# OpenRobotLab/EmbodiedScan

Hardware: NVIDIA H100
Metric: training scans/sec mv-3ddet 20-view (ResNet-50/16 + MinkResNet34, 480x640, 100k pts) (higher is better)
Workload: dtype bf16

## Files before the change

### embodiedscan_b200/csrc/common.cuh

```cuda
#pragma once
#include <cuda_runtime.h>
#include <cuda_bf16.h>
#include <stdint.h>
#include <stdio.h>
#include <stdarg.h>
#include "../../include/esb200.h"

void esb_set_error(const char* fmt, ...);

#define ESB_CHECK_ARG(cond, ...)                      \
  do {                                                \
    if (!(cond)) {                                    \
      esb_set_error(__VA_ARGS__);                     \
      return ESB_EINVAL;                              \
    }                                                 \
  } while (0)

#define ESB_CUDA_LAUNCH_CHECK(name)                                        \
  do {                                                                     \
    cudaError_t _e = cudaPeekAtLastError();                                \
    if (_e != cudaSuccess) {                                               \
      esb_set_error("%s: CUDA error %s", name, cudaGetErrorString(_e));    \
      return ESB_ECUDA;                                                    \
    }                                                                      \
  } while (0)

#define ESB_CUDA_CALL(expr)                                                \
  do {                                                                     \
    cudaError_t _e = (expr);                                               \
    if (_e != cudaSuccess) {                                               \
      esb_set_error("%s: CUDA error %s", #expr, cudaGetErrorString(_e));   \
      return ESB_ECUDA;                                                    \
    }                                                                      \
  } while (0)

static inline int esb_div_up(long long a, long long b) { return (int)((a + b - 1) / b); }
static inline size_t esb_align(size_t x, size_t a = 256) { return (x + a - 1) / a * a; }
cudaError_t esb_scratch_alloc(void** p, size_t bytes, cudaStream_t s);
cudaError_t esb_scratch_free(void* p, cudaStream_t s);
int esb_sum_partial_rows(const float* part, int n_parts, long long width, float* out, int accumulate, cudaStream_t s);

int esb_sm_count();

template <int MODE>
__device__ __forceinline__ float esb_cd_crit(float x) {
  if constexpr (MODE == ESB_CD_L1) {
    return fabsf(x);
  } else if constexpr (MODE == ESB_CD_L2) {
    return __fmul_rn(x, x);
  } else {
    const float a = fabsf(x);
    return a < 1.f ? __fmul_rn(0.5f * a, a) : a - 0.5f;
  }
}
template <int MODE>
__device__ __forceinline__ float esb_cd_dcrit(float x) {
  if constexpr (MODE == ESB_CD_L1) {
    return x > 0.f ? 1.f : (x < 0.f ? -1.f : 0.f);
  } else if constexpr (MODE == ESB_CD_L2) {
    return 2.f * x;
  } else {
    return fminf(fmaxf(x, -1.f), 1.f);
  }
}


#define ESB_EMPTY_KEY 0xFFFFFFFFFFFFFFFFull
#define ESB_COORD_BIAS 32768

__host__ __device__ __forceinline__ uint64_t esb_pack_key(int b, int x, int y, int z) {
  return ((uint64_t)(uint16_t)b << 48) | ((uint64_t)(uint16_t)(x + ESB_COORD_BIAS) << 32) |
         ((uint64_t)(uint16_t)(y + ESB_COORD_BIAS) << 16) | (uint64_t)(uint16_t)(z + ESB_COORD_BIAS);
}
__host__ __device__ __forceinline__ bool esb_coord_in_range(int b, int x, int y, int z) {
  return b >= 0 && b < 65535 && x >= -ESB_COORD_BIAS && x < ESB_COORD_BIAS && y >= -ESB_COORD_BIAS &&
         y < ESB_COORD_BIAS && z >= -ESB_COORD_BIAS && z < ESB_COORD_BIAS;
}
__host__ __device__ __forceinline__ uint32_t esb_hash64(uint64_t k) {
  k ^= k >> 33;
  k *= 0xff51afd7ed558ccdull;
  k ^= k >> 33;
  k *= 0xc4ceb9fe1a85ec53ull;
  k ^= k >> 33;
  return (uint32_t)k;
}

#ifdef __CUDACC__
__device__ __forceinline__ int esb_floor_div(int a, int d) {
  int q = a / d;
  return (a % d != 0 && a < 0) ? q - 1 : q;
}

__device__ __forceinline__ int esb_hash_find(const unsigned long long* __restrict__ keys,
                                             const int* __restrict__ vals, uint32_t mask, uint64_t key) {
  uint32_t slot = esb_hash64(key) & mask;
  for (uint32_t probe = 0; probe <= mask; ++probe) {
    unsigned long long k = keys[slot];
    if (k == key) return vals[slot];
    if (k == ESB_EMPTY_KEY) return -1;
    slot = (slot + 1) & mask;
  }
  return -1;
}

template <typename T>
__device__ __forceinline__ float esb_to_float(T v);
template <>
__device__ __forceinline__ float esb_to_float<float>(float v) { return v; }
template <>
__device__ __forceinline__ float esb_to_float<__nv_bfloat16>(__nv_bfloat16 v) { return __bfloat162float(v); }

template <typename T>
__device__ __forceinline__ T esb_from_float(float v);
template <>
__device__ __forceinline__ float esb_from_float<float>(float v) { return v; }
template <>
__device__ __forceinline__ __nv_bfloat16 esb_from_float<__nv_bfloat16>(float v) { return __float2bfloat16_rn(v); }

__device__ __forceinline__ float esb_warp_sum(float v) {
#pragma unroll
  for (int o = 16; o > 0; o >>= 1) v += __shfl_xor_sync(0xffffffffu, v, o);
  return v;
}
__device__ __forceinline__ float esb_warp_max(float v) {
#pragma unroll
  for (int o = 16; o > 0; o >>= 1) v = fmaxf(v, __shfl_xor_sync(0xffffffffu, v, o));
  return v;
}
#endif
```

### embodiedscan_b200/csrc/scratch.cu

```cuda
#include <mutex>

#include "common.cuh"

namespace {

__global__ void sum_partial_rows_kernel(const float* __restrict__ part, int n_parts, long long width, float* __restrict__ out,
                                        int accumulate) {
  const long long j = blockIdx.x * (long long)blockDim.x + threadIdx.x;
  if (j >= width) return;
  float s = accumulate ? out[j] : 0.f;
  for (int p = 0; p < n_parts; ++p) s += part[(long long)p * width + j];
  out[j] = s;
}

}

int esb_sm_count() {
  static int sms[64] = {};
  int dev = 0;
  cudaGetDevice(&dev);
  if (dev >= 64) return 132;
  if (sms[dev] == 0) {
    int n = 132;
    cudaDeviceGetAttribute(&n, cudaDevAttrMultiProcessorCount, dev);
    sms[dev] = n;
  }
  return sms[dev];
}

namespace {
constexpr unsigned long long kScratchKeepBytes = 512ull << 20;
std::mutex g_pool_mutex;
cudaMemPool_t g_pool[64] = {};

cudaMemPool_t scratch_pool(int dev, cudaStream_t s) {
  if (dev < 0 || dev >= 64) return nullptr;
  std::lock_guard<std::mutex> lock(g_pool_mutex);
  if (g_pool[dev] == nullptr) {
    cudaStreamCaptureStatus st = cudaStreamCaptureStatusNone;
    cudaStreamIsCapturing(s, &st);
    if (st != cudaStreamCaptureStatusNone) return nullptr;
    cudaMemPoolProps props = {};
    props.allocType = cudaMemAllocationTypePinned;
    props.location.type = cudaMemLocationTypeDevice;
    props.location.id = dev;
    cudaMemPool_t pool = nullptr;
    if (cudaMemPoolCreate(&pool, &props) != cudaSuccess) return nullptr;
    unsigned long long keep = kScratchKeepBytes;
    cudaMemPoolSetAttribute(pool, cudaMemPoolAttrReleaseThreshold, &keep);
    g_pool[dev] = pool;
  }
  return g_pool[dev];
}
}

cudaError_t esb_scratch_alloc(void** p, size_t bytes, cudaStream_t s) {
  int dev = 0;
  cudaGetDevice(&dev);
  const size_t n = bytes > 0 ? bytes : 16;
  cudaMemPool_t pool = scratch_pool(dev, s);
  return pool != nullptr ? cudaMallocFromPoolAsync(p, n, pool, s) : cudaMallocAsync(p, n, s);
}

cudaError_t esb_scratch_free(void* p, cudaStream_t s) { return cudaFreeAsync(p, s); }

int esb_sum_partial_rows(const float* part, int n_parts, long long width, float* out, int accumulate, cudaStream_t s) {
  if (width == 0) return ESB_OK;
  sum_partial_rows_kernel<<<esb_div_up(width, 256), 256, 0, s>>>(part, n_parts, width, out, accumulate);
  ESB_CUDA_LAUNCH_CHECK("sum_partial_rows_kernel");
  return ESB_OK;
}
```

### embodiedscan_b200/csrc/spops.cu

```cuda
#include "common.cuh"

namespace {

template <typename T>
__global__ void maxpool_fwd_kernel(const T* __restrict__ x, const int* __restrict__ nbr, T* __restrict__ y,
                                   int* __restrict__ arg, long long n_out, int C, int K) {
  long long t = blockIdx.x * (long long)blockDim.x + threadIdx.x;
  if (t >= n_out * C) return;
  long long o = t / C;
  int c = (int)(t - o * C);
  float best = -INFINITY;
  int best_i = -1;
  for (int k = 0; k < K; ++k) {
    int i = nbr[(long long)k * n_out + o];
    if (i < 0) continue;
    float v = esb_to_float<T>(x[(long long)i * C + c]);
    if (best_i < 0 || v > best) {
      best = v;
      best_i = i;
    }
  }
  y[t] = esb_from_float<T>(best_i >= 0 ? best : 0.f);
  arg[t] = best_i;
}

template <typename T>
__global__ void maxpool_bwd_kernel(const T* __restrict__ dy, const int* __restrict__ arg, T* __restrict__ dx,
                                   long long n_out, int C) {
  long long t = blockIdx.x * (long long)blockDim.x + threadIdx.x;
  if (t >= n_out * C) return;
  int c = (int)(t % C);
  int i = arg[t];
  if (i >= 0) dx[(long long)i * C + c] = dy[t];
}

__device__ __forceinline__ int seg_begin(const int* __restrict__ seg_off, int s) { return seg_off ? seg_off[s] : 0; }
__device__ __forceinline__ int seg_end(const int* __restrict__ seg_off, int s, int n_total) {
  return seg_off ? seg_off[s + 1] : n_total;
}

template <typename T, int MODE>
__global__ void seg_colstat_kernel(const T* __restrict__ x, const int* __restrict__ seg_off, const float* __restrict__ mean,
                                   float* __restrict__ out, int C, int rows_per_block, int n_total) {
  __shared__ float red[8][33];
  const int s = blockIdx.y;
  const int c = blockIdx.z * 32 + threadIdx.x;
  const int r_beg = seg_begin(seg_off, s) + blockIdx.x * rows_per_block;
  const int r_end = min(seg_end(seg_off, s, n_total), r_beg + rows_per_block);
  float acc = 0.f;
  if (c < C) {
    float mu = MODE == 1 ? mean[s * C + c] : 0.f;
    for (int r = r_beg + threadIdx.y; r < r_end; r += 8) {
      float v = esb_to_float<T>(x[(long long)r * C + c]);
      if (MODE == 1) {
        v -= mu;
        acc = fmaf(v, v, acc);
      } else {
        acc += v;
      }
    }
  }
  red[threadIdx.y][threadIdx.x] = acc;
  __syncthreads();
  if (threadIdx.y == 0 && c < C) {
    float t = 0.f;
#pragma unroll
    for (int j = 0; j < 8; ++j) t += red[j][threadIdx.x];
    out[((long long)blockIdx.x * gridDim.y + s) * C + c] = t;
  }
}

__global__ void seg_finalize_mean_kernel(float* __restrict__ sum, const int* __restrict__ seg_off, int S, int C,
                                         int n_total) {
  int t = blockIdx.x * blockDim.x + threadIdx.x;
  if (t >= S * C) return;
  int s = t / C;
  int n = seg_end(seg_off, s, n_total) - seg_begin(seg_off, s);
  sum[t] = n > 0 ? sum[t] / (float)n : 0.f;
}
__global__ void seg_finalize_rstd_kernel(const float* __restrict__ mean, float* __restrict__ var_to_rstd,
                                         const int* __restrict__ seg_off, int S, int C, float eps,
                                         float* __restrict__ running_mean, float* __restrict__ running_var,
                                         float momentum, int n_total) {
  int t = blockIdx.x * blockDim.x + threadIdx.x;
  if (t >= S * C) return;
  int s = t / C;
  int n = seg_end(seg_off, s, n_total) - seg_begin(seg_off, s);
  float var = n > 0 ? var_to_rstd[t] / (float)n : 0.f;
  if (running_mean != nullptr && S == 1) {
    float unbiased = n > 1 ? var * (float)n / (float)(n - 1) : var;
    running_mean[t] = (1.f - momentum) * running_mean[t] + momentum * mean[t];
    running_var[t] = (1.f - momentum) * running_var[t] + momentum * unbiased;
  }
  var_to_rstd[t] = rsqrtf(var + eps);
}

__device__ __forceinline__ float act_fwd(float z, int act) {
  if (act == 1) return fmaxf(z, 0.f);
  if (act == 2) return z > 0.f ? z : expm1f(z);
  return z;
}
__device__ __forceinline__ float act_bwd_from_out(float y, int act) {
  if (act == 1) return y > 0.f ? 1.f : 0.f;
  if (act == 2) return y > 0.f ? 1.f : y + 1.f;
  return 1.f;
}

template <typename T>
__global__ void norm_apply_kernel(const T* __restrict__ x, const T* __restrict__ res, const int* __restrict__ row_seg,
                                  const float* __restrict__ mean, const float* __restrict__ rstd,
                                  const float* __restrict__ gamma, const float* __restrict__ beta, T* __restrict__ y,
                                  long long N, int C, int act) {
  long long t = blockIdx.x * (long long)blockDim.x + threadIdx.x;
  if (t >= N * C) return;
  long long r = t / C;
  int c = (int)(t - r * C);
  int s = row_seg ? row_seg[r] : 0;
  float g = gamma ? gamma[c] : 1.f, b = beta ? beta[c] : 0.f;
  float z = (esb_to_float<T>(x[t]) - mean[s * C + c]) * rstd[s * C + c] * g + b;
  if (res) z += esb_to_float<T>(res[t]);
  y[t] = esb_from_float<T>(act_fwd(z, act));
}

template <typename T>
__device__ __forceinline__ void load8(const T* p, float v[8]);
template <>
__device__ __forceinline__ void load8<float>(const float* p, float v[8]) {
  float4 a = reinterpret_cast<const float4*>(p)[0], b = reinterpret_cast<const float4*>(p)[1];
  v[0] = a.x; v[1] = a.y; v[2] = a.z; v[3] = a.w; v[4] = b.x; v[5] = b.y; v[6] = b.z; v[7] = b.w;
}
template <>
__device__ __forceinline__ void load8<__nv_bfloat16>(const __nv_bfloat16* p, float v[8]) {
  uint4 raw = *reinterpret_cast<const uint4*>(p);
  const __nv_bfloat162* h = reinterpret_cast<const __nv_bfloat162*>(&raw);
#pragma unroll
  for (int i = 0; i < 4; ++i) { v[2 * i] = __low2float(h[i]); v[2 * i + 1] = __high2float(h[i]); }
}
template <typename T>
__device__ __forceinline__ void store8(T* p, const float v[8]);
template <>
__device__ __forceinline__ void store8<float>(float* p, const float v[8]) {
  reinterpret_cast<float4*>(p)[0] = make_float4(v[0], v[1], v[2], v[3]);
  reinterpret_cast<float4*>(p)[1] = make_float4(v[4], v[5], v[6], v[7]);
}
template <>
__device__ __forceinline__ void store8<__nv_bfloat16>(__nv_bfloat16* p, const float v[8]) {
  uint4 o;
  __nv_bfloat162* h = reinterpret_cast<__nv_bfloat162*>(&o);
#pragma unroll
  for (int i = 0; i < 4; ++i) h[i] = __floats2bfloat162_rn(v[2 * i], v[2 * i + 1]);
  *reinterpret_cast<uint4*>(p) = o;
}

template <typename T>
__global__ void norm_apply_vec8_kernel(const T* __restrict__ x, const T* __restrict__ res, const int* __restrict__ row_seg,
                                       const float* __restrict__ mean, const float* __restrict__ rstd,
                                       const float* __restrict__ gamma, const float* __restrict__ beta, T* __restrict__ y,
                                       long long n_vec, int C, int act) {
  long long t = blockIdx.x * (long long)blockDim.x + threadIdx.x;
  if (t >= n_vec) return;
  const int cv = C >> 3;
  const long long r = t / cv;
  const int c0 = (int)(t - r * cv) << 3;
  const int s = row_seg ? row_seg[r] : 0;
  float v[8], rr[8];
  load8<T>(x + t * 8, v);
  if (res) load8<T>(res + t * 8, rr);
#pragma unroll
  for (int i = 0; i < 8; ++i) {
    const int c = c0 + i;
    float z = (v[i] - mean[s * C + c]) * rstd[s * C + c] * (gamma ? gamma[c] : 1.f) + (beta ? beta[c] : 0.f);
    if (res) z += rr[i];
    v[i] = act_fwd(z, act);
  }
  store8<T>(y + t * 8, v);
}

template <typename T>
__global__ void norm_bwd_apply_vec8_kernel(const T* __restrict__ x, const T* __restrict__ y, const T* __restrict__ dy,
                                           const int* __restrict__ row_seg, const int* __restrict__ seg_off,
                                           const float* __restrict__ mean, const float* __restrict__ rstd,
                                           const float* __restrict__ gamma, const float* __restrict__ sg,
                                           const float* __restrict__ sgx, T* __restrict__ dx, T* __restrict__ dres,
                                           long long N, long long n_vec, int C, int act) {
  long long t = blockIdx.x * (long long)blockDim.x + threadIdx.x;
  if (t >= n_vec) return;
  const int cv = C >> 3;
  const long long r = t / cv;
  const int c0 = (int)(t - r * cv) << 3;
  const int s = row_seg ? row_seg[r] : 0;
  const float inv_n = 1.f / (float)max(seg_end(seg_off, s, (int)N) - seg_begin(seg_off, s), 1);
  float xv[8], yv[8], gv[8], ov[8];
  load8<T>(x + t * 8, xv);
  load8<T>(y + t * 8, yv);
  load8<T>(dy + t * 8, gv);
#pragma unroll
  for (int i = 0; i < 8; ++i) {
    const int c = c0 + i;
    float g = gv[i] * act_bwd_from_out(yv[i], act);
    float rs = rstd[s * C + c];
    float xh = (xv[i] - mean[s * C + c]) * rs;
    ov[i] = (gamma ? gamma[c] : 1.f) * rs * (g - sg[s * C + c] * inv_n - xh * sgx[s * C + c] * inv_n);
    gv[i] = g;
  }
  store8<T>(dx + t * 8, ov);
  if (dres) store8<T>(dres + t * 8, gv);
}

template <typename T>
__global__ void norm_bwd_reduce_kernel(const T* __restrict__ x, const T* __restrict__ y, const T* __restrict__ dy,
                                       const int* __restrict__ seg_off, const float* __restrict__ mean,
                                       const float* __restrict__ rstd, float* __restrict__ sg, float* __restrict__ sgx,
                                       int C, int rows_per_block, int act, int n_total) {
  __shared__ float red0[8][33];
  __shared__ float red1[8][33];
  const int s = blockIdx.y;
  const int c = blockIdx.z * 32 + threadIdx.x;
  const int r_beg = seg_begin(seg_off, s) + blockIdx.x * rows_per_block;
  const int r_end = min(seg_end(seg_off, s, n_total), r_beg + rows_per_block);
  float a0 = 0.f, a1 = 0.f;
  if (c < C) {
    float mu = mean[s * C + c], rs = rstd[s * C + c];
    for (int r = r_beg + threadIdx.y; r < r_end; r += 8) {
      long long idx = (long long)r * C + c;
      float g = esb_to_float<T>(dy[idx]) * act_bwd_from_out(esb_to_float<T>(y[idx]), act);
      float xh = (esb_to_float<T>(x[idx]) - mu) * rs;
      a0 += g;
      a1 = fmaf(g, xh, a1);
    }
  }
  red0[threadIdx.y][threadIdx.x] = a0;
  red1[threadIdx.y][threadIdx.x] = a1;
  __syncthreads();
  if (threadIdx.y == 0 && c < C) {
    float t0 = 0.f, t1 = 0.f;
#pragma unroll
    for (int j = 0; j < 8; ++j) {
      t0 += red0[j][threadIdx.x];
      t1 += red1[j][threadIdx.x];
    }
    sg[((long long)blockIdx.x * gridDim.y + s) * C + c] = t0;
    sgx[((long long)blockIdx.x * gridDim.y + s) * C + c] = t1;
  }
}

template <typename T>
__global__ void norm_bwd_apply_kernel(const T* __restrict__ x, const T* __restrict__ y, const T* __restrict__ dy,
                                      const int* __restrict__ row_seg, const int* __restrict__ seg_off,
                                      const float* __restrict__ mean, const float* __restrict__ rstd,
                                      const float* __restrict__ gamma, const float* __restrict__ sg,
                                      const float* __restrict__ sgx, T* __restrict__ dx, T* __restrict__ dres,
                                      long long N, int C, int act) {
  long long t = blockIdx.x * (long long)blockDim.x + threadIdx.x;
  if (t >= N * C) return;
  long long r = t / C;
  int c = (int)(t - r * C);
  int s = row_seg ? row_seg[r] : 0;
  float inv_n = 1.f / (float)max(seg_end(seg_off, s, (int)N) - seg_begin(seg_off, s), 1);
  float g = esb_to_float<T>(dy[t]) * act_bwd_from_out(esb_to_float<T>(y[t]), act);
  float rs = rstd[s * C + c];
  float xh = (esb_to_float<T>(x[t]) - mean[s * C + c]) * rs;
  float gm = gamma ? gamma[c] : 1.f;
  float v = gm * rs * (g - sg[s * C + c] * inv_n - xh * sgx[s * C + c] * inv_n);
  dx[t] = esb_from_float<T>(v);
  if (dres) dres[t] = esb_from_float<T>(g);
}

template <typename T>
__global__ void bias_act_kernel(const T* __restrict__ x, const float* __restrict__ bias, const T* __restrict__ res,
                                T* __restrict__ y, long long n_vec, int C, int act) {
  long long t = blockIdx.x * (long long)blockDim.x + threadIdx.x;
  if (t >= n_vec) return;
  const int cv = C / 8;
  const int c0 = (int)(t % cv) * 8;
  float v[8], r[8];
  if (sizeof(T) == 2) {
    uint4 raw = reinterpret_cast<const uint4*>(x)[t];
    const __nv_bfloat162* h = reinterpret_cast<const __nv_bfloat162*>(&raw);
#pragma unroll
    for (int i = 0; i < 4; ++i) { v[2 * i] = __low2float(h[i]); v[2 * i + 1] = __high2float(h[i]); }
    if (res) {
      uint4 rr = reinterpret_cast<const uint4*>(res)[t];
      const __nv_bfloat162* g = reinterpret_cast<const __nv_bfloat162*>(&rr);
#pragma unroll
      for (int i = 0; i < 4; ++i) { r[2 * i] = __low2float(g[i]); r[2 * i + 1] = __high2float(g[i]); }
    }
  } else {
#pragma unroll
    for (int i = 0; i < 8; ++i) { v[i] = esb_to_float<T>(x[t * 8 + i]); r[i] = res ? esb_to_float<T>(res[t * 8 + i]) : 0.f; }
  }
#pragma unroll
  for (int i = 0; i < 8; ++i) v[i] = act_fwd(v[i] + (bias ? bias[c0 + i] : 0.f) + (res ? r[i] : 0.f), act);
  if (sizeof(T) == 2) {
    uint4 o;
    __nv_bfloat162* h = reinterpret_cast<__nv_bfloat162*>(&o);
#pragma unroll
    for (int i = 0; i < 4; ++i) h[i] = __floats2bfloat162_rn(v[2 * i], v[2 * i + 1]);
    reinterpret_cast<uint4*>(y)[t] = o;
  } else {
#pragma unroll
    for (int i = 0; i < 8; ++i) y[t * 8 + i] = esb_from_float<T>(v[i]);
  }
}

template <typename T>
__global__ void act_bwd_kernel(const T* __restrict__ dy, const T* __restrict__ y, T* __restrict__ dx, long long n,
                               int act) {
  long long t = (blockIdx.x * (long long)blockDim.x + threadIdx.x) * 8;
  if (t + 8 <= n) {
    float g[8], o[8];
    load8<T>(dy + t, g);
    load8<T>(y + t, o);
#pragma unroll
    for (int i = 0; i < 8; ++i) g[i] *= act_bwd_from_out(o[i], act);
    store8<T>(dx + t, g);
  } else {
    for (int i = 0; i < 8; ++i)
      if (t + i < n)
        dx[t + i] = esb_from_float<T>(esb_to_float<T>(dy[t + i]) * act_bwd_from_out(esb_to_float<T>(y[t + i]), act));
  }
}

template <typename T>
__global__ void bn_stats_kernel(const T* __restrict__ x, long long N, int C, int rows_per_block, float* __restrict__ part) {
  extern __shared__ float sh[];
  const int tpr = C / 8;
  const int c = (threadIdx.x % tpr) * 8;
  const int rsub = threadIdx.x / tpr, rstep = blockDim.x / tpr;
  const long long r_beg = (long long)blockIdx.x * rows_per_block;
  const long long r_end = r_beg + rows_per_block < N ? r_beg + rows_per_block : N;
  float piv[8], sum[8], sq[8];
  load8<T>(x + c, piv);
#pragma unroll
  for (int e = 0; e < 8; ++e) sum[e] = sq[e] = 0.f;
  if (rsub < rstep) {
    for (long long r = r_beg + rsub; r < r_end; r += rstep) {
      float v[8];
      load8<T>(x + r * C + c, v);
#pragma unroll
      for (int e = 0; e < 8; ++e) {
        const float d = v[e] - piv[e];
        sum[e] += d;
        sq[e] = fmaf(d, d, sq[e]);
      }
    }
#pragma unroll
    for (int e = 0; e < 8; ++e) {
      sh[(2 * rsub) * C + c + e] = sum[e];
      sh[(2 * rsub + 1) * C + c + e] = sq[e];
    }
  }
  __syncthreads();
  for (int i = threadIdx.x; i < 2 * C; i += blockDim.x) {
    const int k = i < C ? 0 : 1, ci = i < C ? i : i - C;
    float t = 0.f;
    for (int r = 0; r < rstep; ++r) t += sh[(2 * r + k) * C + ci];
    part[(long long)blockIdx.x * 2 * C + i] = t;
  }
}

template <typename T>
__global__ void bn_apply_fused_kernel(const T* __restrict__ x, const T* __restrict__ res, long long N, int C,
                                      const float* __restrict__ gamma, const float* __restrict__ beta, float eps,
                                      float* __restrict__ running_mean, float* __restrict__ running_var, float momentum, int act,
                                      float* __restrict__ stats, T* __restrict__ y) {
  const float inv_n = 1.f / (float)N;
  if (blockIdx.x == 0) {
    for (int i = threadIdx.x; i < C; i += blockDim.x) {
      const float m = stats[i] * inv_n;
      const float var = fmaxf(stats[C + i] * inv_n - m * m, 0.f);
      const float mean = esb_to_float<T>(x[i]) + m;
      stats[2 * C + i] = mean;
      stats[3 * C + i] = rsqrtf(var + eps);
      if (running_mean != nullptr) {
        const float unbiased = N > 1 ? var * (float)N / (float)(N - 1) : var;
        running_mean[i] = (1.f - momentum) * running_mean[i] + momentum * mean;
        running_var[i] = (1.f - momentum) * running_var[i] + momentum * unbiased;
      }
    }
  }
  const long long t = blockIdx.x * (long long)blockDim.x + threadIdx.x;
  const int cv = C / 8;
  if (t >= N * cv) return;
  const long long r = t / cv;
  const int c = (int)(t - r * cv) * 8;
  float v[8], piv[8], rs[8];
  load8<T>(x + r * C + c, v);
  load8<T>(x + c, piv);
  if (res != nullptr) load8<T>(res + r * C + c, rs);
#pragma unroll
  for (int e = 0; e < 8; ++e) {
    const float m = stats[c + e] * inv_n;
    const float var = fmaxf(stats[C + c + e] * inv_n - m * m, 0.f);
    const float g = gamma ? gamma[c + e] : 1.f, b = beta ? beta[c + e] : 0.f;
    float z = (v[e] - (piv[e] + m)) * rsqrtf(var + eps) * g + b;
    if (res != nullptr) z += rs[e];
    v[e] = act_fwd(z, act);
  }
  store8<T>(y + r * C + c, v);
}

template <typename T>
__global__ void gather2_rows_kernel(const T* __restrict__ a, const int* __restrict__ ia, long long na, const T* __restrict__ b,
                                    const int* __restrict__ ib, T* __restrict__ out, long long n_vec, int C) {
  const long long i = (long long)blockIdx.x * blockDim.x + threadIdx.x;
  if (i >= n_vec) return;
  const int cv = C / 8;
  const long long r = i / cv;
  const int c = (int)(i - r * cv) * 8;
  const long long ra = ia ? (long long)ia[r] : (r < na ? r : -1);
  float v[8];
#pragma unroll
  for (int e = 0; e < 8; ++e) v[e] = 0.f;
  if (ra >= 0) load8<T>(a + ra * C + c, v);
  if (b != nullptr) {
    const int rb = ib[r];
    if (rb >= 0) {
      float w[8];
      load8<T>(b + (long long)rb * C + c, w);
#pragma unroll
      for (int e = 0; e < 8; ++e) v[e] += w[e];
    }
  }
  store8<T>(out + r * C + c, v);
}

}

#define DISPATCH_T(dtype, ...)                         \
  if (dtype == ESB_F32) {                              \
    using T = float;                                   \
    __VA_ARGS__;                                       \
  } else {                                             \
    using T = __nv_bfloat16;                           \
    __VA_ARGS__;                                       \
  }

extern "C" int esb_maxpool_fwd(const void* x, const int* nbr, void* y, int* arg, long long n_out, int C, int K,
                               int dtype, void* stream) {
  if (n_out == 0) return ESB_OK;
  DISPATCH_T(dtype, (maxpool_fwd_kernel<T><<<esb_div_up(n_out * C, 256), 256, 0, (cudaStream_t)stream>>>(
                        (const T*)x, nbr, (T*)y, arg, n_out, C, K)));
  ESB_CUDA_LAUNCH_CHECK("maxpool_fwd_kernel");
  return ESB_OK;
}

extern "C" int esb_maxpool_bwd(const void* dy, const int* arg, void* dx, long long n_out, int C, int dtype,
                               void* stream) {
  if (n_out == 0) return ESB_OK;
  DISPATCH_T(dtype, (maxpool_bwd_kernel<T><<<esb_div_up(n_out * C, 256), 256, 0, (cudaStream_t)stream>>>(
                        (const T*)dy, arg, (T*)dx, n_out, C)));
  ESB_CUDA_LAUNCH_CHECK("maxpool_bwd_kernel");
  return ESB_OK;
}

extern "C" int esb_norm_fwd(const void* x, const void* res, const int* seg_off, const int* row_seg, int S,
                            long long N, int max_seg_rows, int C, const float* gamma, const float* beta, float eps,
                            float* running_mean, float* running_var, float momentum, int act, float* mean, float* rstd,
                            void* y, int dtype, void* stream_) {
  cudaStream_t stream = (cudaStream_t)stream_;
  ESB_CHECK_ARG(S >= 1 && C >= 1, "esb_norm_fwd: bad S/C");
  ESB_CHECK_ARG(seg_off != nullptr || S == 1, "esb_norm_fwd: seg_off may be NULL only for a single segment");
  ESB_CUDA_CALL(cudaMemsetAsync(mean, 0, sizeof(float) * S * C, stream));
  ESB_CUDA_CALL(cudaMemsetAsync(rstd, 0, sizeof(float) * S * C, stream));
  if (N == 0) return ESB_OK;
  const int rpb = 256;
  dim3 grid(esb_div_up(max_seg_rows > 0 ? max_seg_rows : 1, rpb), S, esb_div_up(C, 32)), block(32, 8);
  int fin = esb_div_up(S * C, 256);
  float* part = nullptr;
  ESB_CUDA_CALL(esb_scratch_alloc((void**)&part, sizeof(float) * grid.x * S * C, stream));
  int rc = ESB_OK;
  DISPATCH_T(dtype, {
    seg_colstat_kernel<T, 0><<<grid, block, 0, stream>>>((const T*)x, seg_off, nullptr, part, C, rpb, (int)N);
    rc = esb_sum_partial_rows(part, (int)grid.x, (long long)S * C, mean, 0, stream);
    seg_finalize_mean_kernel<<<fin, 256, 0, stream>>>(mean, seg_off, S, C, (int)N);
    seg_colstat_kernel<T, 1><<<grid, block, 0, stream>>>((const T*)x, seg_off, mean, part, C, rpb, (int)N);
    if (rc == ESB_OK) rc = esb_sum_partial_rows(part, (int)grid.x, (long long)S * C, rstd, 0, stream);
    seg_finalize_rstd_kernel<<<fin, 256, 0, stream>>>(mean, rstd, seg_off, S, C, eps, running_mean, running_var, momentum,
                                                      (int)N);
    if (C % 8 == 0)
      norm_apply_vec8_kernel<T><<<esb_div_up(N * (C / 8), 256), 256, 0, stream>>>(
          (const T*)x, (const T*)res, row_seg, mean, rstd, gamma, beta, (T*)y, N * (C / 8), C, act);
    else
      norm_apply_kernel<T><<<esb_div_up(N * C, 256), 256, 0, stream>>>((const T*)x, (const T*)res, row_seg, mean, rstd,
                                                                       gamma, beta, (T*)y, N, C, act);
  });
  ESB_CUDA_CALL(esb_scratch_free(part, stream));
  if (rc != ESB_OK) return rc;
  ESB_CUDA_LAUNCH_CHECK("esb_norm_fwd");
  return ESB_OK;
}

extern "C" int esb_norm_apply(const void* x, const void* res, const int* row_seg, long long N, int C,
                              const float* mean, const float* rstd, const float* gamma, const float* beta, int act,
                              void* y, int dtype, void* stream) {
  if (N == 0) return ESB_OK;
  DISPATCH_T(dtype, (norm_apply_kernel<T><<<esb_div_up(N * C, 256), 256, 0, (cudaStream_t)stream>>>(
                        (const T*)x, (const T*)res, row_seg, mean, rstd, gamma, beta, (T*)y, N, C, act)));
  ESB_CUDA_LAUNCH_CHECK("norm_apply_kernel");
  return ESB_OK;
}

extern "C" int esb_norm_bwd(const void* x, const void* y, const void* dy, const int* seg_off, const int* row_seg, int S,
                            long long N, int max_seg_rows, int C, const float* mean, const float* rstd,
                            const float* gamma, int act, float* sg, float* sgx, void* dx, void* dres, int zero_sums,
                            int dtype, void* stream_) {
  cudaStream_t stream = (cudaStream_t)stream_;
  if (zero_sums) {
    ESB_CUDA_CALL(cudaMemsetAsync(sg, 0, sizeof(float) * S * C, stream));
    ESB_CUDA_CALL(cudaMemsetAsync(sgx, 0, sizeof(float) * S * C, stream));
  }
  if (N == 0) return ESB_OK;
  const int rpb = 256;
  dim3 grid(esb_div_up(max_seg_rows > 0 ? max_seg_rows : 1, rpb), S, esb_div_up(C, 32)), block(32, 8);
  const long long width = (long long)S * C;
  float* part = nullptr;
  ESB_CUDA_CALL(esb_scratch_alloc((void**)&part, sizeof(float) * 2 * grid.x * width, stream));
  int rc = ESB_OK;
  DISPATCH_T(dtype, {
    norm_bwd_reduce_kernel<T><<<grid, block, 0, stream>>>((const T*)x, (const T*)y, (const T*)dy, seg_off, mean, rstd,
                                                          part, part + grid.x * width, C, rpb, act, (int)N);
    rc = esb_sum_partial_rows(part, (int)grid.x, width, sg, 1, stream);
    if (rc == ESB_OK) rc = esb_sum_partial_rows(part + grid.x * width, (int)grid.x, width, sgx, 1, stream);
    if (C % 8 == 0)
      norm_bwd_apply_vec8_kernel<T><<<esb_div_up(N * (C / 8), 256), 256, 0, stream>>>(
          (const T*)x, (const T*)y, (const T*)dy, row_seg, seg_off, mean, rstd, gamma, sg, sgx, (T*)dx, (T*)dres, N,
          N * (C / 8), C, act);
    else
      norm_bwd_apply_kernel<T><<<esb_div_up(N * C, 256), 256, 0, stream>>>(
          (const T*)x, (const T*)y, (const T*)dy, row_seg, seg_off, mean, rstd, gamma, sg, sgx, (T*)dx, (T*)dres, N, C, act);
  });
  ESB_CUDA_CALL(esb_scratch_free(part, stream));
  if (rc != ESB_OK) return rc;
  ESB_CUDA_LAUNCH_CHECK("esb_norm_bwd");
  return ESB_OK;
}

extern "C" int esb_bias_act_fwd(const void* x, const float* bias, const void* res, void* y, long long rows, int C, int act,
                                int dtype, void* stream) {
  ESB_CHECK_ARG(C % 8 == 0, "esb_bias_act_fwd: C must be a multiple of 8");
  long long n_vec = rows * (C / 8);
  if (n_vec == 0) return ESB_OK;
  DISPATCH_T(dtype, (bias_act_kernel<T><<<esb_div_up(n_vec, 256), 256, 0, (cudaStream_t)stream>>>(
                        (const T*)x, bias, (const T*)res, (T*)y, n_vec, C, act)));
  ESB_CUDA_LAUNCH_CHECK("bias_act_kernel");
  return ESB_OK;
}

extern "C" int esb_act_bwd(const void* dy, const void* y, void* dx, long long n, int act, int dtype, void* stream) {
  if (n == 0) return ESB_OK;
  DISPATCH_T(dtype, (act_bwd_kernel<T><<<esb_div_up(n, 256 * 8), 256, 0, (cudaStream_t)stream>>>(
                        (const T*)dy, (const T*)y, (T*)dx, n, act)));
  ESB_CUDA_LAUNCH_CHECK("act_bwd_kernel");
  return ESB_OK;
}

extern "C" int esb_gather2_rows(const void* a, const int* ia, long long na, const void* b, const int* ib, void* out, long long n,
                                int C, int dtype, void* stream) {
  ESB_CHECK_ARG(C > 0 && C % 8 == 0, "esb_gather2_rows: C must be a positive multiple of 8");
  ESB_CHECK_ARG((b == nullptr) == (ib == nullptr), "esb_gather2_rows: b and ib go together");
  const long long n_vec = n * (C / 8);
  if (n_vec == 0) return ESB_OK;
  DISPATCH_T(dtype, (gather2_rows_kernel<T><<<esb_div_up(n_vec, 256), 256, 0, (cudaStream_t)stream>>>(
                        (const T*)a, ia, na, (const T*)b, ib, (T*)out, n_vec, C)));
  ESB_CUDA_LAUNCH_CHECK("gather2_rows_kernel");
  return ESB_OK;
}

extern "C" int esb_batchnorm_fwd_fused(const void* x, const void* res, long long N, int C, const float* gamma, const float* beta,
                                       float eps, float* running_mean, float* running_var, float momentum, int act, float* stats,
                                       void* y, int dtype, void* stream_) {
  cudaStream_t stream = (cudaStream_t)stream_;
  ESB_CHECK_ARG(C % 8 == 0 && C >= 8 && C <= 2048, "esb_batchnorm_fwd_fused: C must be a multiple of 8 in [8, 2048]");
  ESB_CUDA_CALL(cudaMemsetAsync(stats, 0, sizeof(float) * 2 * C, stream));
  if (N == 0) return ESB_OK;
  long long rpb = (N + 2 * esb_sm_count() - 1) / (2 * esb_sm_count());
  if (rpb < 64) rpb = 64;
  const int grid_a = esb_div_up(N, rpb);
  const long long n_vec = N * (C / 8);
  const int rstep = 256 / (C / 8);
  float* part = nullptr;
  ESB_CUDA_CALL(esb_scratch_alloc((void**)&part, sizeof(float) * 2 * C * grid_a, stream));
  DISPATCH_T(dtype, (bn_stats_kernel<T><<<grid_a, 256, 2 * rstep * C * sizeof(float), stream>>>((const T*)x, N, C, (int)rpb, part)));
  ESB_CUDA_LAUNCH_CHECK("bn_stats_kernel");
  int rc = esb_sum_partial_rows(part, grid_a, 2LL * C, stats, 0, stream);
  ESB_CUDA_CALL(esb_scratch_free(part, stream));
  if (rc != ESB_OK) return rc;
  DISPATCH_T(dtype, (bn_apply_fused_kernel<T><<<esb_div_up(n_vec, 256), 256, 0, stream>>>(
                        (const T*)x, (const T*)res, N, C, gamma, beta, eps, running_mean, running_var, momentum, act, stats,
                        (T*)y)));
  ESB_CUDA_LAUNCH_CHECK("bn_apply_fused_kernel");
  return ESB_OK;
}
```

Baseline: 55.48.

## Fuse norm partial-sum reductions via last-block tickets and grid-stride apply kernels

Replaces the separate memset and sum-partial-rows launches in norm forward/backward and batchnorm with in-kernel finalisation: finalize kernels sum partials directly, and the backward reduce and bn_stats kernels use a per-stream atomic ticket so the last block reduces the partials. The apply kernels become persistent grid-stride kernels sized by occupancy, caching per-segment mean/rstd and gamma/beta in registers. This cuts kernel launches and redundant parameter loads, at the cost of a per-stream ticket counter, a mutex-protected map lookup on every call, and a serial last-block reduction that may bottleneck for wide C.

```diff
diff --git a/embodiedscan_b200/csrc/common.cuh b/embodiedscan_b200/csrc/common.cuh
--- a/embodiedscan_b200/csrc/common.cuh
+++ b/embodiedscan_b200/csrc/common.cuh
@@ -39,6 +39,7 @@
 cudaError_t esb_scratch_alloc(void** p, size_t bytes, cudaStream_t s);
 cudaError_t esb_scratch_free(void* p, cudaStream_t s);
 int esb_sum_partial_rows(const float* part, int n_parts, long long width, float* out, int accumulate, cudaStream_t s);
+unsigned int* esb_stream_ticket(cudaStream_t s);
 
 int esb_sm_count();
 
diff --git a/embodiedscan_b200/csrc/scratch.cu b/embodiedscan_b200/csrc/scratch.cu
--- a/embodiedscan_b200/csrc/scratch.cu
+++ b/embodiedscan_b200/csrc/scratch.cu
@@ -1,4 +1,6 @@
+#include <map>
 #include <mutex>
+#include <utility>
 
 #include "common.cuh"
 
@@ -64,6 +66,20 @@
 
 cudaError_t esb_scratch_free(void* p, cudaStream_t s) { return cudaFreeAsync(p, s); }
 
+unsigned int* esb_stream_ticket(cudaStream_t s) {
+  static std::mutex mutex;
+  static std::map<std::pair<int, cudaStream_t>, unsigned int*> tickets;
+  int dev = 0;
+  cudaGetDevice(&dev);
+  std::lock_guard<std::mutex> lock(mutex);
+  unsigned int*& t = tickets[{dev, s}];
+  if (t == nullptr) {
+    if (cudaMalloc((void**)&t, sizeof(unsigned int)) != cudaSuccess) return t = nullptr;
+    cudaMemsetAsync(t, 0, sizeof(unsigned int), s);
+  }
+  return t;
+}
+
 int esb_sum_partial_rows(const float* part, int n_parts, long long width, float* out, int accumulate, cudaStream_t s) {
   if (width == 0) return ESB_OK;
   sum_partial_rows_kernel<<<esb_div_up(width, 256), 256, 0, s>>>(part, n_parts, width, out, accumulate);
diff --git a/embodiedscan_b200/csrc/spops.cu b/embodiedscan_b200/csrc/spops.cu
--- a/embodiedscan_b200/csrc/spops.cu
+++ b/embodiedscan_b200/csrc/spops.cu
@@ -1,3 +1,5 @@
+#include <algorithm>
+
 #include "common.cuh"
 
 namespace {
@@ -70,29 +72,48 @@
   }
 }
 
-__global__ void seg_finalize_mean_kernel(float* __restrict__ sum, const int* __restrict__ seg_off, int S, int C,
-                                         int n_total) {
-  int t = blockIdx.x * blockDim.x + threadIdx.x;
+__device__ __forceinline__ float chain_sum(const float* part, int P, long long W, long long j) {
+  float s = 0.f;
+#pragma unroll 16
+  for (int p = 0; p < P; ++p) s += __ldcg(part + p * W + j);
+  return s;
+}
+
+__device__ __forceinline__ bool last_block(unsigned int* ticket) {
+  __shared__ bool last;
+  __threadfence();
+  __syncthreads();
+  if (threadIdx.x == 0) last = atomicAdd(ticket, 1u) == gridDim.x * gridDim.y * gridDim.z - 1;
+  __syncthreads();
+  if (last) __threadfence();
+  return last;
+}
+
+__global__ void seg_finalize_mean_kernel(const float* __restrict__ part, int n_parts, const int* __restrict__ seg_off, int S,
+                                         int C, int n_total, float* __restrict__ mean) {
+  const int t = blockIdx.x * blockDim.x + threadIdx.x;
   if (t >= S * C) return;
-  int s = t / C;
-  int n = seg_end(seg_off, s, n_total) - seg_begin(seg_off, s);
-  sum[t] = n > 0 ? sum[t] / (float)n : 0.f;
-}
-__global__ void seg_finalize_rstd_kernel(const float* __restrict__ mean, float* __restrict__ var_to_rstd,
-                                         const int* __restrict__ seg_off, int S, int C, float eps,
+  const int s = t / C;
+  const int n = seg_end(seg_off, s, n_total) - seg_begin(seg_off, s);
+  const float sum = chain_sum(part, n_parts, (long long)S * C, t);
+  mean[t] = n > 0 ? sum / (float)n : 0.f;
+}
+__global__ void seg_finalize_rstd_kernel(const float* __restrict__ part, int n_parts, const float* __restrict__ mean,
+                                         float* __restrict__ rstd, const int* __restrict__ seg_off, int S, int C, float eps,
                                          float* __restrict__ running_mean, float* __restrict__ running_var,
                                          float momentum, int n_total) {
-  int t = blockIdx.x * blockDim.x + threadIdx.x;
+  const int t = blockIdx.x * blockDim.x + threadIdx.x;
   if (t >= S * C) return;
-  int s = t / C;
-  int n = seg_end(seg_off, s, n_total) - seg_begin(seg_off, s);
-  float var = n > 0 ? var_to_rstd[t] / (float)n : 0.f;
+  const int s = t / C;
+  const int n = seg_end(seg_off, s, n_total) - seg_begin(seg_off, s);
+  const float sum = chain_sum(part, n_parts, (long long)S * C, t);
+  const float var = n > 0 ? sum / (float)n : 0.f;
   if (running_mean != nullptr && S == 1) {
     float unbiased = n > 1 ? var * (float)n / (float)(n - 1) : var;
     running_mean[t] = (1.f - momentum) * running_mean[t] + momentum * mean[t];
     running_var[t] = (1.f - momentum) * running_var[t] + momentum * unbiased;
   }
-  var_to_rstd[t] = rsqrtf(var + eps);
+  rstd[t] = rsqrtf(var + eps);
 }
 
 __device__ __forceinline__ float act_fwd(float z, int act) {
@@ -152,96 +173,181 @@
   *reinterpret_cast<uint4*>(p) = o;
 }
 
-template <typename T>
-__global__ void norm_apply_vec8_kernel(const T* __restrict__ x, const T* __restrict__ res, const int* __restrict__ row_seg,
-                                       const float* __restrict__ mean, const float* __restrict__ rstd,
-                                       const float* __restrict__ gamma, const float* __restrict__ beta, T* __restrict__ y,
-                                       long long n_vec, int C, int act) {
-  long long t = blockIdx.x * (long long)blockDim.x + threadIdx.x;
-  if (t >= n_vec) return;
-  const int cv = C >> 3;
-  const long long r = t / cv;
-  const int c0 = (int)(t - r * cv) << 3;
-  const int s = row_seg ? row_seg[r] : 0;
-  float v[8], rr[8];
-  load8<T>(x + t * 8, v);
-  if (res) load8<T>(res + t * 8, rr);
+struct RowSlice {
+  int rstep, rsub, cl, c;
+};
+__device__ __forceinline__ RowSlice row_slice(int C, int slice) {
+  RowSlice t;
+  const int tpr = min((C + 7) >> 3, 256);
+  t.rstep = blockDim.x / tpr;
+  t.rsub = threadIdx.x / tpr;
+  t.cl = threadIdx.x - t.rsub * tpr;
+  t.c = (slice * tpr + t.cl) * 8;
+  return t;
+}
+
+template <typename T>
+__global__ void __launch_bounds__(256) norm_apply_vec8_kernel(const T* __restrict__ x, const T* __restrict__ res,
+                                                              const int* __restrict__ row_seg, const float* __restrict__ mean,
+                                                              const float* __restrict__ rstd, const float* __restrict__ gamma,
+                                                              const float* __restrict__ beta, T* __restrict__ y, long long N,
+                                                              int C, int act) {
+  const RowSlice t = row_slice(C, blockIdx.y);
+  if (t.rsub >= t.rstep || t.c >= C) return;
+  float gm[8], bt[8], mu[8], rs[8];
 #pragma unroll
   for (int i = 0; i < 8; ++i) {
-    const int c = c0 + i;
-    float z = (v[i] - mean[s * C + c]) * rstd[s * C + c] * (gamma ? gamma[c] : 1.f) + (beta ? beta[c] : 0.f);
-    if (res) z += rr[i];
-    v[i] = act_fwd(z, act);
-  }
-  store8<T>(y + t * 8, v);
-}
-
-template <typename T>
-__global__ void norm_bwd_apply_vec8_kernel(const T* __restrict__ x, const T* __restrict__ y, const T* __restrict__ dy,
-                                           const int* __restrict__ row_seg, const int* __restrict__ seg_off,
-                                           const float* __restrict__ mean, const float* __restrict__ rstd,
-                                           const float* __restrict__ gamma, const float* __restrict__ sg,
-                                           const float* __restrict__ sgx, T* __restrict__ dx, T* __restrict__ dres,
-                                           long long N, long long n_vec, int C, int act) {
-  long long t = blockIdx.x * (long long)blockDim.x + threadIdx.x;
-  if (t >= n_vec) return;
-  const int cv = C >> 3;
-  const long long r = t / cv;
-  const int c0 = (int)(t - r * cv) << 3;
-  const int s = row_seg ? row_seg[r] : 0;
-  const float inv_n = 1.f / (float)max(seg_end(seg_off, s, (int)N) - seg_begin(seg_off, s), 1);
-  float xv[8], yv[8], gv[8], ov[8];
-  load8<T>(x + t * 8, xv);
-  load8<T>(y + t * 8, yv);
-  load8<T>(dy + t * 8, gv);
-#pragma unroll
-  for (int i = 0; i < 8; ++i) {
-    const int c = c0 + i;
-    float g = gv[i] * act_bwd_from_out(yv[i], act);
-    float rs = rstd[s * C + c];
-    float xh = (xv[i] - mean[s * C + c]) * rs;
-    ov[i] = (gamma ? gamma[c] : 1.f) * rs * (g - sg[s * C + c] * inv_n - xh * sgx[s * C + c] * inv_n);
-    gv[i] = g;
-  }
-  store8<T>(dx + t * 8, ov);
-  if (dres) store8<T>(dres + t * 8, gv);
-}
-
-template <typename T>
-__global__ void norm_bwd_reduce_kernel(const T* __restrict__ x, const T* __restrict__ y, const T* __restrict__ dy,
-                                       const int* __restrict__ seg_off, const float* __restrict__ mean,
-                                       const float* __restrict__ rstd, float* __restrict__ sg, float* __restrict__ sgx,
-                                       int C, int rows_per_block, int act, int n_total) {
-  __shared__ float red0[8][33];
-  __shared__ float red1[8][33];
-  const int s = blockIdx.y;
-  const int c = blockIdx.z * 32 + threadIdx.x;
-  const int r_beg = seg_begin(seg_off, s) + blockIdx.x * rows_per_block;
-  const int r_end = min(seg_end(seg_off, s, n_total), r_beg + rows_per_block);
-  float a0 = 0.f, a1 = 0.f;
-  if (c < C) {
-    float mu = mean[s * C + c], rs = rstd[s * C + c];
-    for (int r = r_beg + threadIdx.y; r < r_end; r += 8) {
-      long long idx = (long long)r * C + c;
-      float g = esb_to_float<T>(dy[idx]) * act_bwd_from_out(esb_to_float<T>(y[idx]), act);
-      float xh = (esb_to_float<T>(x[idx]) - mu) * rs;
-      a0 += g;
-      a1 = fmaf(g, xh, a1);
-    }
-  }
-  red0[threadIdx.y][threadIdx.x] = a0;
-  red1[threadIdx.y][threadIdx.x] = a1;
+    gm[i] = gamma ? gamma[t.c + i] : 1.f;
+    bt[i] = beta ? beta[t.c + i] : 0.f;
+  }
+  int s_cur = -1;
+  for (long long r = (long long)blockIdx.x * t.rstep + t.rsub; r < N; r += (long long)gridDim.x * t.rstep) {
+    const int s = row_seg ? row_seg[r] : 0;
+    if (s != s_cur) {
+#pragma unroll
+      for (int i = 0; i < 8; ++i) {
+        mu[i] = mean[s * C + t.c + i];
+        rs[i] = rstd[s * C + t.c + i];
+      }
+      s_cur = s;
+    }
+    float v[8], rr[8];
+    load8<T>(x + r * C + t.c, v);
+    if (res) load8<T>(res + r * C + t.c, rr);
+#pragma unroll
+    for (int i = 0; i < 8; ++i) {
+      float z = __fadd_rn(__fmul_rn(__fmul_rn(v[i] - mu[i], rs[i]), gm[i]), bt[i]);
+      if (res) z += rr[i];
+      v[i] = act_fwd(z, act);
+    }
+    store8<T>(y + r * C + t.c, v);
+  }
+}
+
+template <typename T>
+__global__ void __launch_bounds__(256) norm_bwd_apply_vec8_kernel(const T* __restrict__ x, const T* __restrict__ y,
+                                                                  const T* __restrict__ dy, const int* __restrict__ row_seg,
+                                                                  const int* __restrict__ seg_off,
+                                                                  const float* __restrict__ mean, const float* __restrict__ rstd,
+                                                                  const float* __restrict__ gamma, const float* __restrict__ sg,
+                                                                  const float* __restrict__ sgx, T* __restrict__ dx,
+                                                                  T* __restrict__ dres, long long N, int C, int act) {
+  const RowSlice t = row_slice(C, blockIdx.y);
+  if (t.rsub >= t.rstep || t.c >= C) return;
+  float gm[8], mu[8], rs[8], sgv[8], sgxv[8], inv_n = 0.f;
+#pragma unroll
+  for (int i = 0; i < 8; ++i) gm[i] = gamma ? gamma[t.c + i] : 1.f;
+  int s_cur = -1;
+  for (long long r = (long long)blockIdx.x * t.rstep + t.rsub; r < N; r += (long long)gridDim.x * t.rstep) {
+    const int s = row_seg ? row_seg[r] : 0;
+    if (s != s_cur) {
+      inv_n = 1.f / (float)max(seg_end(seg_off, s, (int)N) - seg_begin(seg_off, s), 1);
+#pragma unroll
+      for (int i = 0; i < 8; ++i) {
+        mu[i] = mean[s * C + t.c + i];
+        rs[i] = rstd[s * C + t.c + i];
+        sgv[i] = sg[s * C + t.c + i];
+        sgxv[i] = sgx[s * C + t.c + i];
+      }
+      s_cur = s;
+    }
+    float xv[8], yv[8], gv[8], ov[8];
+    load8<T>(x + r * C + t.c, xv);
+    load8<T>(y + r * C + t.c, yv);
+    load8<T>(dy + r * C + t.c, gv);
+#pragma unroll
+    for (int i = 0; i < 8; ++i) {
+      float g = gv[i] * act_bwd_from_out(yv[i], act);
+      float xh = (xv[i] - mu[i]) * rs[i];
+      ov[i] = gm[i] * rs[i] * (g - sgv[i] * inv_n - xh * sgxv[i] * inv_n);
+      gv[i] = g;
+    }
+    store8<T>(dx + r * C + t.c, ov);
+    if (dres) store8<T>(dres + r * C + t.c, gv);
+  }
+}
+
+template <typename T>
+__global__ void __launch_bounds__(256) norm_bwd_reduce_kernel(const T* __restrict__ x, const T* __restrict__ y,
+                                                              const T* __restrict__ dy, const int* __restrict__ seg_off,
+                                                              const float* __restrict__ mean, const float* __restrict__ rstd,
+                                                              float* __restrict__ part, unsigned int* __restrict__ ticket,
+                                                              float* __restrict__ sg, float* __restrict__ sgx, int C,
+                                                              int n_row_blocks, int act, int n_total, int accumulate) {
+  __shared__ float lanes[2 * 256 * 8];
+  const int s = blockIdx.y, S = gridDim.y;
+  const int tpr = min((C + 7) >> 3, 32);
+  const int per_rb = 8 * tpr, rb_per_cta = 256 / per_rb;
+  const int v = threadIdx.x / per_rb, lane = (threadIdx.x / tpr) & 7, cl = threadIdx.x % tpr;
+  const int width = min(C - (int)blockIdx.z * 256, 256);
+  const int c0 = blockIdx.z * 256 + cl * 8;
+  const int rb = blockIdx.x * rb_per_cta + v;
+  const int r_beg = seg_begin(seg_off, s) + rb * 256;
+  const int r_end = min(seg_end(seg_off, s, n_total), r_beg + 256);
+  float a0[8], a1[8];
+#pragma unroll
+  for (int i = 0; i < 8; ++i) a0[i] = a1[i] = 0.f;
+  if (v < rb_per_cta && rb < n_row_blocks && c0 < C) {
+    float mu[8], rs[8];
+#pragma unroll
+    for (int i = 0; i < 8; ++i) {
+      mu[i] = c0 + i < C ? mean[s * C + c0 + i] : 0.f;
+      rs[i] = c0 + i < C ? rstd[s * C + c0 + i] : 0.f;
+    }
+    for (int r = r_beg + lane; r < r_end; r += 8) {
+      const long long idx = (long long)r * C + c0;
+      float xv[8], yv[8], gv[8];
+      if (C % 8 == 0) {
+        load8<T>(x + idx, xv);
+        load8<T>(y + idx, yv);
+        load8<T>(dy + idx, gv);
+      } else {
+#pragma unroll
+        for (int i = 0; i < 8; ++i) {
+          const bool in = c0 + i < C;
+          xv[i] = in ? esb_to_float<T>(x[idx + i]) : 0.f;
+          yv[i] = in ? esb_to_float<T>(y[idx + i]) : 0.f;
+          gv[i] = in ? esb_to_float<T>(dy[idx + i]) : 0.f;
+        }
+      }
+#pragma unroll
+      for (int i = 0; i < 8; ++i) {
+        const float g = gv[i] * act_bwd_from_out(yv[i], act);
+        const float xh = (xv[i] - mu[i]) * rs[i];
+        a0[i] += g;
+        a1[i] = fmaf(g, xh, a1[i]);
+      }
+    }
+  }
+  const int sw = tpr * 8;
+  float* mine = lanes + v * 16 * sw;
+  if (v < rb_per_cta) {
+#pragma unroll
+    for (int i = 0; i < 8; ++i) {
+      mine[(2 * lane) * sw + cl * 8 + i] = a0[i];
+      mine[(2 * lane + 1) * sw + cl * 8 + i] = a1[i];
+    }
+  }
   __syncthreads();
-  if (threadIdx.y == 0 && c < C) {
-    float t0 = 0.f, t1 = 0.f;
-#pragma unroll
-    for (int j = 0; j < 8; ++j) {
-      t0 += red0[j][threadIdx.x];
-      t1 += red1[j][threadIdx.x];
-    }
-    sg[((long long)blockIdx.x * gridDim.y + s) * C + c] = t0;
-    sgx[((long long)blockIdx.x * gridDim.y + s) * C + c] = t1;
-  }
+  const long long W = 2LL * S * C;
+  for (int i = threadIdx.x; i < rb_per_cta * 2 * width; i += blockDim.x) {
+    const int vb = i / (2 * width), k = (i / width) & 1, ci = i % width;
+    const int b = blockIdx.x * rb_per_cta + vb;
+    if (b >= n_row_blocks) continue;
+    const float* l = lanes + vb * 16 * sw;
+    float t = 0.f;
+#pragma unroll
+    for (int j = 0; j < 8; ++j) t += l[(2 * j + k) * sw + ci];
+    part[b * W + ((long long)k * S + s) * C + blockIdx.z * 256 + ci] = t;
+  }
+  if (!last_block(ticket)) return;
+  const long long SC = (long long)S * C;
+  for (long long j = threadIdx.x; j < W; j += blockDim.x) {
+    const float total = chain_sum(part, n_row_blocks, W, j);
+    float* out = j < SC ? sg + j : sgx + (j - SC);
+    *out = accumulate ? *out + total : total;
+  }
+  if (threadIdx.x == 0) *ticket = 0u;
 }
 
 template <typename T>
@@ -322,8 +428,11 @@
 }
 
 template <typename T>
-__global__ void bn_stats_kernel(const T* __restrict__ x, long long N, int C, int rows_per_block, float* __restrict__ part) {
-  extern __shared__ float sh[];
+__global__ void __launch_bounds__(256) bn_stats_kernel(const T* __restrict__ x, long long N, int C, int rows_per_block,
+                                                       float* __restrict__ part, unsigned int* __restrict__ ticket, float eps,
+                                                       float* __restrict__ running_mean, float* __restrict__ running_var,
+                                                       float momentum, float* __restrict__ stats) {
+  __shared__ float sh[2 * 256 * 8];
   const int tpr = C / 8;
   const int c = (threadIdx.x % tpr) * 8;
   const int rsub = threadIdx.x / tpr, rstep = blockDim.x / tpr;
@@ -357,28 +466,30 @@
     for (int r = 0; r < rstep; ++r) t += sh[(2 * r + k) * C + ci];
     part[(long long)blockIdx.x * 2 * C + i] = t;
   }
+  if (!last_block(ticket)) return;
+  for (int j = threadIdx.x; j < 2 * C; j += blockDim.x) stats[j] = chain_sum(part, gridDim.x, 2LL * C, j);
+  __syncthreads();
+  const float inv_n = 1.f / (float)N;
+  for (int i = threadIdx.x; i < C; i += blockDim.x) {
+    const float m = stats[i] * inv_n;
+    const float var = fmaxf(__fmaf_rn(stats[C + i], inv_n, -__fmul_rn(m, m)), 0.f);
+    const float mean = __fadd_rn(esb_to_float<T>(x[i]), m);
+    stats[2 * C + i] = mean;
+    stats[3 * C + i] = rsqrtf(var + eps);
+    if (running_mean != nullptr) {
+      const float unbiased = N > 1 ? var * (float)N / (float)(N - 1) : var;
+      running_mean[i] = (1.f - momentum) * running_mean[i] + momentum * mean;
+      running_var[i] = (1.f - momentum) * running_var[i] + momentum * unbiased;
+    }
+  }
+  if (threadIdx.x == 0) *ticket = 0u;
 }
 
 template <typename T>
 __global__ void bn_apply_fused_kernel(const T* __restrict__ x, const T* __restrict__ res, long long N, int C,
-                                      const float* __restrict__ gamma, const float* __restrict__ beta, float eps,
-                                      float* __restrict__ running_mean, float* __restrict__ running_var, float momentum, int act,
-                                      float* __restrict__ stats, T* __restrict__ y) {
+                                      const float* __restrict__ gamma, const float* __restrict__ beta, float eps, int act,
+                                      const float* __restrict__ stats, T* __restrict__ y) {
   const float inv_n = 1.f / (float)N;
-  if (blockIdx.x == 0) {
-    for (int i = threadIdx.x; i < C; i += blockDim.x) {
-      const float m = stats[i] * inv_n;
-      const float var = fmaxf(stats[C + i] * inv_n - m * m, 0.f);
-      const float mean = esb_to_float<T>(x[i]) + m;
-      stats[2 * C + i] = mean;
-      stats[3 * C + i] = rsqrtf(var + eps);
-      if (running_mean != nullptr) {
-        const float unbiased = N > 1 ? var * (float)N / (float)(N - 1) : var;
-        running_mean[i] = (1.f - momentum) * running_mean[i] + momentum * mean;
-        running_var[i] = (1.f - momentum) * running_var[i] + momentum * unbiased;
-      }
-    }
-  }
   const long long t = blockIdx.x * (long long)blockDim.x + threadIdx.x;
   const int cv = C / 8;
   if (t >= N * cv) return;
@@ -425,6 +536,20 @@
   store8<T>(out + r * C + c, v);
 }
 
+int slice_rows(int C) { return 256 / std::min((C + 7) / 8, 256); }
+int slice_count(int C) { return esb_div_up(esb_div_up(C, 8), 256); }
+
+template <typename Kernel>
+int stream_blocks(Kernel kernel, int& resident_per_sm, long long N, int C) {
+  if (resident_per_sm == 0) {
+    int n = 0;
+    cudaOccupancyMaxActiveBlocksPerMultiprocessor(&n, kernel, 256, 0);
+    resident_per_sm = std::max(n, 1);
+  }
+  const long long need = esb_div_up(N, slice_rows(C));
+  return (int)std::min<long long>(need, (long long)resident_per_sm * esb_sm_count());
+}
+
 }
 
 #define DISPATCH_T(dtype, ...)                         \
@@ -461,32 +586,32 @@
   cudaStream_t stream = (cudaStream_t)stream_;
   ESB_CHECK_ARG(S >= 1 && C >= 1, "esb_norm_fwd: bad S/C");
   ESB_CHECK_ARG(seg_off != nullptr || S == 1, "esb_norm_fwd: seg_off may be NULL only for a single segment");
-  ESB_CUDA_CALL(cudaMemsetAsync(mean, 0, sizeof(float) * S * C, stream));
-  ESB_CUDA_CALL(cudaMemsetAsync(rstd, 0, sizeof(float) * S * C, stream));
-  if (N == 0) return ESB_OK;
+  if (N == 0) {
+    ESB_CUDA_CALL(cudaMemsetAsync(mean, 0, sizeof(float) * S * C, stream));
+    ESB_CUDA_CALL(cudaMemsetAsync(rstd, 0, sizeof(float) * S * C, stream));
+    return ESB_OK;
+  }
   const int rpb = 256;
   dim3 grid(esb_div_up(max_seg_rows > 0 ? max_seg_rows : 1, rpb), S, esb_div_up(C, 32)), block(32, 8);
-  int fin = esb_div_up(S * C, 256);
+  const int fin = esb_div_up((long long)S * C, 256);
+  static int occ[2] = {};
   float* part = nullptr;
   ESB_CUDA_CALL(esb_scratch_alloc((void**)&part, sizeof(float) * grid.x * S * C, stream));
-  int rc = ESB_OK;
   DISPATCH_T(dtype, {
     seg_colstat_kernel<T, 0><<<grid, block, 0, stream>>>((const T*)x, seg_off, nullptr, part, C, rpb, (int)N);
-    rc = esb_sum_partial_rows(part, (int)grid.x, (long long)S * C, mean, 0, stream);
-    seg_finalize_mean_kernel<<<fin, 256, 0, stream>>>(mean, seg_off, S, C, (int)N);
+    seg_finalize_mean_kernel<<<fin, 256, 0, stream>>>(part, (int)grid.x, seg_off, S, C, (int)N, mean);
     seg_colstat_kernel<T, 1><<<grid, block, 0, stream>>>((const T*)x, seg_off, mean, part, C, rpb, (int)N);
-    if (rc == ESB_OK) rc = esb_sum_partial_rows(part, (int)grid.x, (long long)S * C, rstd, 0, stream);
-    seg_finalize_rstd_kernel<<<fin, 256, 0, stream>>>(mean, rstd, seg_off, S, C, eps, running_mean, running_var, momentum,
-                                                      (int)N);
+    seg_finalize_rstd_kernel<<<fin, 256, 0, stream>>>(part, (int)grid.x, mean, rstd, seg_off, S, C, eps, running_mean,
+                                                      running_var, momentum, (int)N);
     if (C % 8 == 0)
-      norm_apply_vec8_kernel<T><<<esb_div_up(N * (C / 8), 256), 256, 0, stream>>>(
-          (const T*)x, (const T*)res, row_seg, mean, rstd, gamma, beta, (T*)y, N * (C / 8), C, act);
+      norm_apply_vec8_kernel<T><<<dim3(stream_blocks(norm_apply_vec8_kernel<T>, occ[dtype == ESB_F32], N, C), slice_count(C)), 256,
+                                   0, stream>>>(
+          (const T*)x, (const T*)res, row_seg, mean, rstd, gamma, beta, (T*)y, N, C, act);
     else
       norm_apply_kernel<T><<<esb_div_up(N * C, 256), 256, 0, stream>>>((const T*)x, (const T*)res, row_seg, mean, rstd,
                                                                        gamma, beta, (T*)y, N, C, act);
   });
   ESB_CUDA_CALL(esb_scratch_free(part, stream));
-  if (rc != ESB_OK) return rc;
   ESB_CUDA_LAUNCH_CHECK("esb_norm_fwd");
   return ESB_OK;
 }
@@ -506,32 +631,34 @@
                             const float* gamma, int act, float* sg, float* sgx, void* dx, void* dres, int zero_sums,
                             int dtype, void* stream_) {
   cudaStream_t stream = (cudaStream_t)stream_;
-  if (zero_sums) {
-    ESB_CUDA_CALL(cudaMemsetAsync(sg, 0, sizeof(float) * S * C, stream));
-    ESB_CUDA_CALL(cudaMemsetAsync(sgx, 0, sizeof(float) * S * C, stream));
-  }
-  if (N == 0) return ESB_OK;
-  const int rpb = 256;
-  dim3 grid(esb_div_up(max_seg_rows > 0 ? max_seg_rows : 1, rpb), S, esb_div_up(C, 32)), block(32, 8);
-  const long long width = (long long)S * C;
+  if (N == 0) {
+    if (zero_sums) {
+      ESB_CUDA_CALL(cudaMemsetAsync(sg, 0, sizeof(float) * S * C, stream));
+      ESB_CUDA_CALL(cudaMemsetAsync(sgx, 0, sizeof(float) * S * C, stream));
+    }
+    return ESB_OK;
+  }
+  const long long width = 2LL * S * C;
+  const int n_rb = esb_div_up(max_seg_rows > 0 ? max_seg_rows : 1, 256);
+  const int rb_per_cta = 256 / (8 * std::min((C + 7) / 8, 32));
+  dim3 grid(esb_div_up(n_rb, rb_per_cta), S, esb_div_up(C, 256));
+  unsigned int* ticket = esb_stream_ticket(stream);
+  ESB_CHECK_ARG(ticket != nullptr, "esb_norm_bwd: no ticket counter for this stream");
+  static int occ[2] = {};
   float* part = nullptr;
-  ESB_CUDA_CALL(esb_scratch_alloc((void**)&part, sizeof(float) * 2 * grid.x * width, stream));
-  int rc = ESB_OK;
+  ESB_CUDA_CALL(esb_scratch_alloc((void**)&part, sizeof(float) * n_rb * width, stream));
   DISPATCH_T(dtype, {
-    norm_bwd_reduce_kernel<T><<<grid, block, 0, stream>>>((const T*)x, (const T*)y, (const T*)dy, seg_off, mean, rstd,
-                                                          part, part + grid.x * width, C, rpb, act, (int)N);
-    rc = esb_sum_partial_rows(part, (int)grid.x, width, sg, 1, stream);
-    if (rc == ESB_OK) rc = esb_sum_partial_rows(part + grid.x * width, (int)grid.x, width, sgx, 1, stream);
+    norm_bwd_reduce_kernel<T><<<grid, 256, 0, stream>>>((const T*)x, (const T*)y, (const T*)dy, seg_off, mean, rstd, part,
+                                                        ticket, sg, sgx, C, n_rb, act, (int)N, zero_sums ? 0 : 1);
     if (C % 8 == 0)
-      norm_bwd_apply_vec8_kernel<T><<<esb_div_up(N * (C / 8), 256), 256, 0, stream>>>(
-          (const T*)x, (const T*)y, (const T*)dy, row_seg, seg_off, mean, rstd, gamma, sg, sgx, (T*)dx, (T*)dres, N,
-          N * (C / 8), C, act);
+      norm_bwd_apply_vec8_kernel<T><<<dim3(stream_blocks(norm_bwd_apply_vec8_kernel<T>, occ[dtype == ESB_F32], N, C), slice_count(C)),
+                                      256, 0, stream>>>((const T*)x, (const T*)y, (const T*)dy, row_seg, seg_off, mean, rstd, gamma,
+                                                sg, sgx, (T*)dx, (T*)dres, N, C, act);
     else
       norm_bwd_apply_kernel<T><<<esb_div_up(N * C, 256), 256, 0, stream>>>(
           (const T*)x, (const T*)y, (const T*)dy, row_seg, seg_off, mean, rstd, gamma, sg, sgx, (T*)dx, (T*)dres, N, C, act);
   });
   ESB_CUDA_CALL(esb_scratch_free(part, stream));
-  if (rc != ESB_OK) return rc;
   ESB_CUDA_LAUNCH_CHECK("esb_norm_bwd");
   return ESB_OK;
 }
@@ -572,23 +699,23 @@
                                        void* y, int dtype, void* stream_) {
   cudaStream_t stream = (cudaStream_t)stream_;
   ESB_CHECK_ARG(C % 8 == 0 && C >= 8 && C <= 2048, "esb_batchnorm_fwd_fused: C must be a multiple of 8 in [8, 2048]");
-  ESB_CUDA_CALL(cudaMemsetAsync(stats, 0, sizeof(float) * 2 * C, stream));
-  if (N == 0) return ESB_OK;
+  if (N == 0) {
+    ESB_CUDA_CALL(cudaMemsetAsync(stats, 0, sizeof(float) * 2 * C, stream));
+    return ESB_OK;
+  }
   long long rpb = (N + 2 * esb_sm_count() - 1) / (2 * esb_sm_count());
   if (rpb < 64) rpb = 64;
   const int grid_a = esb_div_up(N, rpb);
-  const long long n_vec = N * (C / 8);
-  const int rstep = 256 / (C / 8);
+  unsigned int* ticket = esb_stream_ticket(stream);
+  ESB_CHECK_ARG(ticket != nullptr, "esb_batchnorm_fwd_fused: no ticket counter for this stream");
   float* part = nullptr;
   ESB_CUDA_CALL(esb_scratch_alloc((void**)&part, sizeof(float) * 2 * C * grid_a, stream));
-  DISPATCH_T(dtype, (bn_stats_kernel<T><<<grid_a, 256, 2 * rstep * C * sizeof(float), stream>>>((const T*)x, N, C, (int)rpb, part)));
+  DISPATCH_T(dtype, (bn_stats_kernel<T><<<grid_a, 256, 0, stream>>>((const T*)x, N, C, (int)rpb, part, ticket, eps, running_mean,
+                                                                    running_var, momentum, stats)));
   ESB_CUDA_LAUNCH_CHECK("bn_stats_kernel");
-  int rc = esb_sum_partial_rows(part, grid_a, 2LL * C, stats, 0, stream);
   ESB_CUDA_CALL(esb_scratch_free(part, stream));
-  if (rc != ESB_OK) return rc;
-  DISPATCH_T(dtype, (bn_apply_fused_kernel<T><<<esb_div_up(n_vec, 256), 256, 0, stream>>>(
-                        (const T*)x, (const T*)res, N, C, gamma, beta, eps, running_mean, running_var, momentum, act, stats,
-                        (T*)y)));
+  DISPATCH_T(dtype, (bn_apply_fused_kernel<T><<<esb_div_up(N * (C / 8), 256), 256, 0, stream>>>(
+                        (const T*)x, (const T*)res, N, C, gamma, beta, eps, act, stats, (T*)y)));
   ESB_CUDA_LAUNCH_CHECK("bn_apply_fused_kernel");
   return ESB_OK;
 }
```

Measured after the change: 56.03, median of 6. About the same (+1.0%).
